# synthesizer-project/synference

Measured on AMD Instinct MI355X. Metric: posterior samples/sec (accepted, prior-box rejection included), higher is better.
Workload: dtype f32

## Files before the change

synference_amd/csrc/sf_api.hip:

```cpp
#include <hip/hip_runtime.h>

#include <chrono>
#include <cmath>
#include <cstdio>
#include <cstdlib>
#include <cstring>
#include <string>
#include <vector>

#include "sf_internal.h"
#include "sf_train.h"
#include "sf_nsf1.h"
#include "sf_nsfar.h"
#include "sf_nsfc.h"
#include "sf_trainc.h"

namespace {
thread_local std::string g_err;

int hip_fail(hipError_t e, const char* what) {
  return sf_fail(SF_ERR_HIP, std::string(what) + ": " + hipGetErrorString(e));
}
}

// ... 209 lines not shown
  add("o_wg0", v.o_wg[0]); add("o_bg0", v.o_bg[0]); add("o_w10", v.o_w1[0]); add("o_b10", v.o_b1[0]);
  add("o_w20", v.o_w2[0]); add("o_b20", v.o_b2[0]); add("o_wg1", v.o_wg[1]); add("o_bg1", v.o_bg[1]);
  add("o_w11", v.o_w1[1]); add("o_b11", v.o_b1[1]); add("o_w21", v.o_w2[1]); add("o_b21", v.o_b2[1]);
  add("o_wout", v.o_wout); add("o_bout", v.o_bout); add("o_lu", v.o_lu);
  add("c_pscale", v.c_pscale); add("c_pshift", v.c_pshift); add("c_tdim", v.c_tdim);
  add("c_xmean", v.c_xmean); add("c_xstd", v.c_xstd); add("c_dslot", v.c_dslot);
  add("nsf_split_sampler", f->L.nsfS.ok); add("trainc_ok", f->L.trc.ok); add("nsfc_ok", f->L.nsc.ok);
  add("inc_ok", v.inc_ok); add("hidden_bf16", v.hidden_bf16); add("tB_stride", v.tB_stride); add("n_parts", v.n_parts); add("part_max", v.part_max);
  add("n_params", f->L.n_params); add("n_packed", f->L.n_packed);
  {
    int R = 0, NV = 0;
    SfDev vv = v;
    vv.packed16 = reinterpret_cast<const float*>(1);
    sf_ctab_shape(vv, R, NV);
    add("ctab_floats_per_galaxy", (long)v.T * NV * R);
  }
  add("o16_w0", v.o16_w0); add("o16_wc", v.o16_wc); add("o16_b0", v.o16_b0); add("o16_wk0", v.o16_wk[0]);
  add("o16_wk1", v.o16_wk[1]); add("o16_bk0", v.o16_bk[0]); add("o16_bk1", v.o16_bk[1]); add("o16_hv", v.o16_hv);
  add("o16_hvb", v.o16_hvb); add("o16_wh", v.o16_wh); add("o16_bh", v.o16_bh); add("o16_wp", v.o16_wp); add("t16_a_tab", v.t16_a_tab);
  add("t16_a", v.t16_a); add("t16B_stride", v.t16B_stride); add("nP16", v.nP16); add("o16B_wk0", v.o16B_wk[0]); add("o16B_wk1", v.o16B_wk[1]);
  add("t16c_stride", v.t16c_stride); add("o16c_bk1", v.o16c_bk1); add("o16c_hvb", v.o16c_hvb); add("o16c_bh", v.o16c_bh);
  add("o16c_wh", v.o16c_wh); add("o16c_wp", v.o16c_wp); add("o16c_blk", v.o16c_blk); add("c16_fix", sf_maf16_compact_fix(v));
  add("sampler_fused", (f->dev_ready && f->ctab_x) ? (sf_maf16_plan(sampler_dev(f, f->ctab_x)).fused ? 1 : 0) : 0);
  add("m16_ok", v.m16_ok); add("m16_span", v.m16_span); add("nT16", v.nT16); add("nC16", v.nC16); add("t16_stride", v.t16_stride);
  s += "\"g16_tile\": [";
  for (int i = 0; i < SF_DMAX; ++i) s += std::to_string(v.g16_tile[i]) + (i + 1 < SF_DMAX ? ", " : "], ");
  s += "\"g16_lo\": [";
  for (int i = 0; i < SF_DMAX; ++i) s += std::to_string(v.g16_lo[i]) + (i + 1 < SF_DMAX ? ", " : "], ");
  s += "\"g_kend\": [";
  for (int i = 0; i < SF_DMAX; ++i) s += std::to_string(v.g_kend[i]) + (i + 1 < SF_DMAX ? ", " : "], ");
  s += "\"g_lo\": [";
  for (int i = 0; i < SF_DMAX; ++i) s += std::to_string(v.g_lo[i]) + (i + 1 < SF_DMAX ? ", " : "], ");
  s += "\"g_tile\": [";
  for (int i = 0; i < SF_DMAX; ++i) s += std::to_string(v.g_tile[i]) + (i + 1 < SF_DMAX ? ", " : "], ");
  s += "\"mt_kend\": [";
  for (int i = 0; i < 4; ++i) s += std::to_string(v.mt_kend[i]) + (i + 1 < 4 ? ", " : "], ");
  s += "\"cst\": [";
  for (size_t i = 0; i < f->L.cst.size(); ++i) {
    char t[40];
    std::snprintf(t, sizeof(t), "%.9g%s", f->L.cst[i], i + 1 < f->L.cst.size() ? ", " : "");
    s += t;
  }
  s += "]}";
  if (s.size() + 1 > buflen) return sf_fail(SF_ERR_INVALID, "buffer too small");
  std::memcpy(buf, s.c_str(), s.size() + 1);
  return SF_OK;
}
// ... 802 lines not shown
```

synference_amd/csrc/sf_layout.cpp:

```cpp
#include "sf_layout.h"

#include <cmath>
#include <cstring>
#include <functional>

namespace {

struct Emitter {
  std::vector<int32_t>& s1;
  std::vector<int32_t>& s2;
  std::vector<int32_t>* gidx = nullptr;
  int64_t cur = 0;

  int64_t pad_to(int64_t align) {
    while (cur % align) push(-1, -1);
    return cur;
  }
  void push(int32_t a, int32_t b, int64_t g = -1) {
    s1.push_back(a);
    s2.push_back(b);
    if (gidx) gidx->push_back((int32_t)(g >= 0 ? g : cur));
    ++cur;
  }
  int64_t linear(int OT, int nG, const std::vector<int>& orow, const std::vector<int>& irow,
// ... 54 lines not shown
  if (d.kind == SF_NSF && (d.K < 2 || d.K > 16)) return fail("K must be in 2..16");
  if (!d.theta_mean || !d.theta_std || !d.x_mean || !d.x_std)
    return fail("z-score buffers must be given");

  const int D = d.D, C = d.C, H = d.H, T = d.T, NB = d.NB, K = d.K;
  SfDev& v = L.dev;
  std::memset(&v, 0, sizeof(v));
  std::memset(&L.trc, 0, sizeof(L.trc));
  std::memset(&L.nsc, 0, sizeof(L.nsc));
  std::memset(&L.nsfS, 0, sizeof(L.nsfS));
  v.kind = d.kind; v.D = D; v.C = C; v.H = H; v.T = T; v.K = K; v.NB = NB;
  v.scale_fn = d.scale_fn;
  v.HT = ceil_div(H, 32);
  v.nGu = ceil_div(D, 8);
  v.nGc = ceil_div(C, 8);
  v.nGh = ceil_div(H, 8);
  v.tail_bound = d.tail_bound; v.min_w = d.min_bin_width; v.min_h = d.min_bin_height;
  v.min_d = d.min_derivative; v.eps = d.maf_eps; v.lu_eps = d.lu_eps;
  v.inv_sqrt_h = (float)(1.0 / std::sqrt((double)H));
  v.deriv_const = (float)std::log(std::exp(1.0 - (double)d.min_derivative) - 1.0);

  std::vector<int> hrow_full(4 * 32, -1);
  std::vector<int> h16row(4 * 16, -1);
  v.inc_ok = 0;
  v.m16_ok = 0;
  if (d.kind == SF_MAF) {
    const int mx = std::max(1, D - 1), mn = std::min(1, D - 1);
    const int G = mx;
    std::vector<std::vector<int>> grp(G);
    for (int j = 0; j < H; ++j) grp[j % mx].push_back(j);
    std::vector<int> rows(4 * 32, -1);
    int tile = 0, used = 0;
    bool ok = true;
    std::vector<int> gt(G), gend(G);
    for (int g = 0; g < G && ok; ++g) {
      const int n = (int)grp[g].size();
      if (n > 32) { ok = false; break; }
      if (used + n > 32) { ++tile; used = 0; }
      if (tile >= 4) { ok = false; break; }
      for (int q = 0; q < n; ++q) rows[tile * 32 + used + q] = grp[g][q];
      used += n;
      gt[g] = tile;
      gend[g] = tile * 32 + used;
    }
    if (ok && D >= 2) {
      const int nGu_e = ceil_div(D, 8), nGc_e = ceil_div(C, 8);
      auto image_floats = [&](int ht, int ngh) {
        return 256L * (ht * (nGu_e + nGc_e) + (long)NB * ht * ngh + ngh) + 64L * D * ht + 64L * (NB + 1) * ht;
// ... 16 lines not shown
      int r = 0;
      for (int g = 0; g < G; ++g) {
        v.g_lo[g + mn] = r / 32;
        for (int j : grp[g]) hrow_full[r++] = j;
        v.g_tile[g + mn] = (r - 1) / 32;
        v.g_kend[g + mn] = ceil_div(r, 8);
      }
      v.inc_ok = (D >= 2 && D <= SF_DMAX && H <= 128) ? 1 : 0;
    }
    {
      h16row.assign(4 * 16, -1);
      int tile16 = 0, used16 = 0;
      bool ok16 = (D >= 2 && NB <= 2);
      for (int g = 0; g < G && ok16; ++g) {
        const int n = (int)grp[g].size();
        if (n > 16) { ok16 = false; break; }
        if (used16 + n > 16) { ++tile16; used16 = 0; }
        if (tile16 >= 4) { ok16 = false; break; }
        for (int q = 0; q < n; ++q) h16row[tile16 * 16 + used16 + q] = grp[g][q];
        used16 += n;
        v.g16_tile[g + mn] = tile16;
      }
      for (int g = 0; g < G; ++g) v.g16_lo[g + mn] = v.g16_tile[g + mn];
      if (!ok16 && D >= 2 && NB <= 2 && H <= 64) {
        h16row.assign(4 * 16, -1);
        int r = 0;
        for (int g = 0; g < G; ++g) {
          v.g16_lo[g + mn] = r / 16;
          for (int j : grp[g]) h16row[r++] = j;
          v.g16_tile[g + mn] = (r - 1) / 16;
        }
        tile16 = (H - 1) / 16;
        ok16 = true;
        v.m16_span = 1;
      }
      v.m16_ok = ok16 ? 1 : 0;
      v.nT16 = ok16 ? tile16 + 1 : 0;
      v.nC16 = ceil_div(C, 16);
    }
  } else {
    for (int j = 0; j < H; ++j) hrow_full[j] = j;
  }
  const int HT = v.HT;
  for (int mt = 0; mt < 4; ++mt) v.mt_kend[mt] = v.nGh;
  if (d.kind == SF_MAF && v.inc_ok) {
    const int mn = std::min(1, D - 1), G = std::max(1, D - 1);
    for (int mt = 0; mt < 4; ++mt) {
      int k = 0;
      for (int g = 0; g < G; ++g)
        if (v.g_lo[g + mn] <= mt && mt <= v.g_tile[g + mn]) k = std::max(k, v.g_kend[g + mn]);
      if (k > 0) v.mt_kend[mt] = k;
    }
  } else if (d.kind == SF_MAF && D >= 2 && H <= 128) {
    const int mx = std::max(1, D - 1);
// ... 276 lines not shown
        if (t == 0) {
          c.ok = 1;
          c.NT = NT;
          std::vector<int> insrc(16, -1);
          int f = 0;
          for (int rho = 0; rho < 16 && f < C; ++rho) {
            const bool slot_row = (rho & 3) < 2 && 2 * (rho >> 2) + (rho & 3) < D;
            if (!slot_row) insrc[rho] = f++;
          }
          while (f < C) {
            for (int rho = 0; rho < 16; ++rho) insrc.push_back(f < C ? f++ : -1);
          }
          c.NI = (int)insrc.size() / 16;
          c.c_insrc = (int)L.cst.size();
          for (int q : insrc) L.cst.push_back((float)q);
          for (int ot = 0; ot < 4; ++ot) { c.kend[ot] = 0; c.kbeg[ot] = NT > 0 ? NT - 1 : 0; }
          c.c_jobs = (int)L.cst.size();
          c.n_jobs = 0;
          for (int ot = 0; ot < NT; ++ot)
            for (int it = 0; it < NT; ++it) {
              bool any = false;
              for (int ro = 0; ro < 16 && !any; ++ro)
                for (int ri = 0; ri < 16 && !any; ++ri) {
                  const int oo = h16row[ot * 16 + ro], ii = h16row[it * 16 + ri];
                  any = oo >= 0 && ii >= 0 && deg_h(oo) >= deg_h(ii);
                }
              if (any) {
                c.kend[ot] = std::max(c.kend[ot], it);
                c.kbeg[it] = std::min(c.kbeg[it], ot);
                L.cst.push_back((float)(ot * 4 + it));
                ++c.n_jobs;
              }
            }
          while (L.cst.size() % 4) L.cst.push_back(0.f);
        }
        const int NI = c.NI;
        auto insrc_at = [&](int it, int rho) { return (int)L.cst[c.c_insrc + it * 16 + rho]; };
        auto pushC = [&](int32_t a, int32_t b) { L.srcC1.push_back(a); L.srcC2.push_back(b); };
        while (L.srcC1.size() % 256) pushC(-1, -1);
        const int64_t tbC = (int64_t)L.srcC1.size();
        if (t == 1) c.t_stride = (int)tbC;
        auto hereC = [&]() { return (int)((int64_t)L.srcC1.size() - tbC); };
        int64_t gcur = 0;
        const int64_t gbase_t = (int64_t)t * c.g_stride;
        auto w_in = [&](int to, int ro, int ti, int ri) -> int64_t {
          const int oo = h16row[to * 16 + ro];
          if (oo < 0) return -1;
          if (ti == 0 && (ri & 3) < 2) {
            const int p = 2 * (ri >> 2) + (ri & 3);
            if (p < D) return deg_h(oo) >= sinv[p] + 1 ? lW0 + (int64_t)oo * D + sinv[p] : -1;
          }
          const int fsrc = insrc_at(ti, ri);
          return fsrc >= 0 ? lWc + (int64_t)oo * C + fsrc : -1;
        };
        auto w_hid = [&](int64_t base) {
          return [&, base](int to, int ro, int ti, int ri) -> int64_t {
            const int oo = h16row[to * 16 + ro], ii = h16row[ti * 16 + ri];
            return (oo >= 0 && ii >= 0 && deg_h(oo) >= deg_h(ii)) ? base + (int64_t)oo * H + ii : -1;
          };
        };
        auto head_row = [&](int ro) -> int {
          const int p = 2 * (ro >> 2) + (ro & 1);
          if (p >= D) return -1;
          return 2 * sinv[p] + ((ro & 3) >= 2 ? 1 : 0);
        };
        auto w_head = [&](int , int ro, int ti, int ri) -> int64_t {
          const int orow_l = head_row(ro), ii = h16row[ti * 16 + ri];
          return (orow_l >= 0 && ii >= 0 && (orow_l / 2 + 1) > deg_h(ii)) ? lWf + (int64_t)orow_l * H + ii : -1;
        };
        using WFn = std::function<int64_t(int, int, int, int)>;
        auto fwd_block = [&](int OT, int IT, const WFn& fn, int64_t g_off) {
          for (int ot = 0; ot < OT; ++ot)
            for (int it = 0; it < IT; ++it)
              for (int l = 0; l < 64; ++l)
                for (int r = 0; r < 4; ++r) {
                  const int ro = l & 15, ri = 4 * (l >> 4) + r;
                  const int64_t idx = fn(ot, ro, it, ri);
                  pushC((int32_t)idx, -1);
                  if (idx >= 0) L.gdstC[(size_t)idx] = (int32_t)(gbase_t + g_off + ((int64_t)ot * IT + it) * 256 + (ro & 3) * 64 + (ro >> 2) * 16 + ri);
                }
        };
        auto tr_block = [&](int ITr, int OTk, const WFn& fn) {
          for (int it = 0; it < ITr; ++it)
            for (int ot = 0; ot < OTk; ++ot)
              for (int l = 0; l < 64; ++l)
                for (int r = 0; r < 4; ++r) pushC((int32_t)fn(ot, 4 * (l >> 4) + r, it, l & 15), -1);
        };
        auto bias_block = [&](int OT, const std::function<int64_t(int, int)>& f1, const std::function<int64_t(int, int)>& f2,
                              int64_t g_off) {
          for (int ot = 0; ot < OT; ++ot)
            for (int ro = 0; ro < 16; ++ro) {
              const int64_t a1 = f1(ot, ro), a2 = f2 ? f2(ot, ro) : -1;
              pushC((int32_t)a1, (int32_t)a2);
              const int32_t g = (int32_t)(gbase_t + g_off + ot * 16 + ro);
              if (a1 >= 0) L.gdstC[(size_t)a1] = g;
              if (a2 >= 0) L.gdstC[(size_t)a2] = g;
            }
        };
        auto hid_bias = [&](int64_t base) {
          return [&, base](int ot, int ro) -> int64_t { const int oo = h16row[ot * 16 + ro]; return oo >= 0 ? base + oo : -1; };
        };
        if (t == 0) L.gdstC.assign((size_t)0, -1);
        if (L.gdstC.size() < (size_t)P) L.gdstC.resize((size_t)P, -1);
        int o; int64_t g;
        o = hereC(); g = gcur; gcur += (int64_t)NT * NI * 256; fwd_block(NT, NI, w_in, g);
        if (t == 0) { c.o_win = o; c.g_win = (int)g; }
        o = hereC(); g = gcur; gcur += NT * 16; bias_block(NT, hid_bias(lb0), hid_bias(lbc), g);
        if (t == 0) { c.o_b0 = o; c.g_b0 = (int)g; }
        o = hereC(); g = gcur; gcur += (int64_t)NT * NT * 256; fwd_block(NT, NT, w_hid(lWk[0]), g);
        if (t == 0) { c.o_w1 = o; c.g_w1 = (int)g; }
        o = hereC(); g = gcur; gcur += NT * 16; bias_block(NT, hid_bias(lbk[0]), nullptr, g);
        if (t == 0) { c.o_b1 = o; c.g_b1 = (int)g; }
        o = hereC(); g = gcur; gcur += (int64_t)NT * NT * 256; fwd_block(NT, NT, w_hid(lWk[1]), g);
        if (t == 0) { c.o_w2 = o; c.g_w2 = (int)g; }
        o = hereC(); g = gcur; gcur += NT * 16; bias_block(NT, hid_bias(lbk[1]), nullptr, g);
        if (t == 0) { c.o_b2 = o; c.g_b2 = (int)g; }
        o = hereC(); g = gcur; gcur += (int64_t)NT * 256; fwd_block(1, NT, w_head, g);
        if (t == 0) { c.o_wf = o; c.g_wf = (int)g; }
        o = hereC(); g = gcur; gcur += 16;
        bias_block(1, [&](int, int ro) -> int64_t { const int r_ = head_row(ro); return r_ >= 0 ? lbf + r_ : -1; }, nullptr, g);
        if (t == 0) { c.o_bf = o; c.g_bf = (int)g; }
        o = hereC(); tr_block(NT, 1, w_head);
        if (t == 0) c.o_wfT = o;
// ... 542 lines not shown
```

synference_amd/csrc/sf_layout.h:

```cpp
#pragma once
#include <cstdint>
#include <string>
#include <vector>

#include "../../include/synference_hip.h"

#define SF_DMAX 16
#define SF_NBMAX 4

struct SfDev {
  const float* packed;
  const float* packedT;
  const float* cst;
  int kind, D, C, H, T, K, NB, scale_fn;
  int HT;
  int PT;
  int KMAX;
  int JP;
  int nGu, nGc, nGh;
  int t_stride;
  int n_parts, part_off[5], part_max;
  int blk_part[SF_NBMAX], head_part;
  int partB_off[5], part_bytes_max;
  int o_w0, o_wc, o_b0;
// ... 10 lines not shown
  int oT_wf, oT_wk[SF_NBMAX], oT_w0;
  int oT_wout, oT_w1[SF_NBMAX], oT_w2[SF_NBMAX], oT_winu;
  int oT_wc;
  int oT_wg[SF_NBMAX];
  int inc_ok;
  int g_tile[SF_DMAX], g_kend[SF_DMAX];
  int g_lo[SF_DMAX];
  int mt_kend[4];
  const unsigned short* packedB;
  int hidden_bf16, nKS, tB_stride;
  int oB_wk[SF_NBMAX], oB_w1[SF_NBMAX], oB_w2[SF_NBMAX];
  const float* packed16;
  int m16_ok, nT16, nC16, t16_stride;
  int t16_a;
  int t16_a_tab;
  int o16_wh, o16_bh;
  int o16_wp;
  const float* packed16c;
  int t16c_stride;
  int o16c_bk1, o16c_hvb, o16c_bh, o16c_wh, o16c_wp, o16c_blk;
  const uint32_t* packed16B;
  int t16B_stride, nP16, o16B_wk[2];
  int m16_span;
  int o16_w0, o16_wc, o16_b0, o16_wk[2], o16_bk[2], o16_hv, o16_hvb;
  int g16_tile[SF_DMAX];
  int g16_lo[SF_DMAX];
  const float* ctab;
  int ctab_R, ctab_NV;
  int c_pscale, c_pshift, c_tdim, c_xmean, c_xstd;
  int c_dslot;
  float logdet0;
  float tail_bound, min_w, min_h, min_d, eps, lu_eps, inv_sqrt_h, deriv_const;
};

#define SF_PACK_TANH_SCALE (-2)
#define SF_PACK_SPLIT_SCALED (1 << 29)
#define SF_PACK_SPLIT_INDEX 0x1fffffff
#define SF_TANH_PRESCALE 2.8853900817779268f

struct SfTrcDev {
  int ok;
  int NT, NI;
  int t_stride, g_stride;
  int o_win, o_b0, o_w1, o_b1, o_w2, o_b2, o_wf, o_bf;
  int o_wfT, o_w2T, o_w1T, o_winT;
  int g_win, g_b0, g_w1, g_b1, g_w2, g_b2, g_wf, g_bf;
// ... 74 lines not shown
```

synference_amd/csrc/sf_maf16.hip:

```cpp
#include "sf_maf16_pass.h"

template <int NB, bool SPAN>
__global__ __launch_bounds__(256, 3) void k_maf_inv16(SfDev m, SfSampleArgsHost a) {
  const int lane = threadIdx.x & 63, wave = threadIdx.x >> 6;
  const int s = lane & 15, g4 = lane >> 4;
  const long item = ((long)blockIdx.x * 4 + wave) * 16 + s;
  const bool valid = item < a.n_items;
  const long it = valid ? item : a.n_items - 1;
  const SfItem16 I = sf_item16(m, a, it, g4);
  f32x4 u = I.u;
  const uint32_t slot = I.slot, att_mine = I.att;
  const long gal = I.gal, ps_idx = I.ps;
  const float* xr = a.x + gal * m.C;
  float logdet = 0.f;

  const float* ctg = (m.ctab && !a.z_in) ? m.ctab + (size_t)gal * m.T * m.ctab_R : nullptr;
  f32x4 ct0;
  if (!ctg) ct0 = sf_ctx_tile16(m, xr, 0, g4);

  const int NT = m.nT16;
  SfPass16 S;
#pragma unroll
  for (int k = 0; k < 3; ++k)
#pragma unroll
// ... 141 lines not shown
           m.o16c_blk == o_blk && m.t16c_stride == size;
  }
  static __device__ __forceinline__ void apply(SfDev& m) {
    m.o16_bk[1] = o_bk1; m.o16_hvb = o_hvb; m.o16_bh = o_bh; m.o16_wh = o_wh; m.o16_wp = o_wp;
  }
};
template <int PREC>
static __host__ __device__ __forceinline__ int sf_lds_floats16(const SfDev& m, bool cp) {
  if constexpr (PREC == 2) return m.t16c_stride + 4 * SF_G16_SCR;
  else return (m.ctab ? m.t16_a_tab : m.t16_a) + SfHid16<PREC>::lds_floats(m, cp);
}
template <int G>
__device__ __forceinline__ void sf_stage16c(const float* src, int wave) {
  const float4* __restrict__ g = reinterpret_cast<const float4*>(src) + (threadIdx.x & 63);
  float4* __restrict__ l = reinterpret_cast<float4*>(sf_lds16);
  for (int gi = __builtin_amdgcn_readfirstlane(wave); gi < G; gi += 4)
    __builtin_amdgcn_global_load_lds((const void*)(g + gi * 64), (void __attribute__((address_space(3)))*)(l + gi * 64), 16, 0, 0);
  __builtin_amdgcn_s_waitcnt(0x0f70);
}

#ifndef SF_SAMP16_WG_FUSED
#define SF_SAMP16_WG_FUSED 4
#endif
template <int NB, bool SPAN, bool HM, int DD = 0, int PREC = 0>
__global__ __launch_bounds__(256, (SPAN ? 3 : (PREC == 2 ? SF_SAMP16_WG_FUSED : 4))) void k_maf_samp16(SfSamp16Args args_in) {
  static_assert(DD == 0 || (HM && !SPAN && DD >= 2 && DD <= 5), "unrolled passes: head tile, aligned placement, D <= 5");
  static_assert(PREC != 2 || DD >= 3, "fused first layer: unrolled kernels only (m_fix and the compact image's offsets)");
  using HID = SfHid16<PREC>;
  constexpr int TPW = SF_SAMP16_TPW;
  constexpr int IPW = 64 * TPW;
  const int wave = threadIdx.x >> 6;
  using FC = SfFixC16<NB, (PREC == 2 ? DD : 2)>;
  unsigned int* ctrl = reinterpret_cast<unsigned int*>(sf_lds16 + sf_lds_floats16<PREC>(args_in.m, !SPAN));
  unsigned int pf;
  sf_q_begin<IPW>(args_in.a, ctrl, pf);
  float* ecb = reinterpret_cast<float*>(ctrl + SF_Q_WORDS(IPW));
  sf_ecb16_build<true>(ecb, args_in.m, args_in.a);
#ifdef SF_Q_STATS
  const unsigned long long qs_k0 = __builtin_amdgcn_s_memtime();
  unsigned long long qs_iters = 0, qs_last_work = 0;
  unsigned long long qs_ph[10] = {0, 0, 0, 0, 0, 0, 0, 0, 0, 0};
  if (threadIdx.x == 0) atomicMin(&args_in.a.q->stats[10], __builtin_amdgcn_s_memrealtime());
#endif
  for (;;) {
    const SfSamp16Args* ap;
    {
      auto kp = __builtin_amdgcn_kernarg_segment_ptr();
      asm volatile("" : "+s"(kp));
// ... 67 lines not shown
      { const unsigned long long n = __builtin_amdgcn_s_memrealtime(); qs_ph[qs_o + (t == m.T - 1 ? 1 : 3)] += n - qs_t_mark; qs_t_mark = n; }
#endif
      __syncthreads();
      if constexpr (PREC == 2) sf_stage16c<FC::groups>(m.packed16c + (size_t)t * FC::size, wave);
      else sf_stage16<PREC, !SPAN>(m, t, S.tab ? m.t16_a_tab : m.t16_a, wave);
      __syncthreads();
#ifdef SF_Q_STATS
      { const unsigned long long n = __builtin_amdgcn_s_memrealtime(); qs_ph[qs_o + 2] += n - qs_t_mark; qs_t_mark = n; }
#endif
      const float* tp = sf_lds16;
      const void* tpB = sf_lds16 + (PREC == 2 ? FC::o_blk : (S.tab ? m.t16_a_tab : m.t16_a));
#pragma unroll 1
      for (int j = 0; j < TPW; ++j) {
        const bool tile_has_work = (unsigned)((j * 4 + wave) * 16) < n_items;
        if (tile_has_work) {
          if (j > 0) {
            S.c0p = S.tab ? m.ctab + ((size_t)gal_cur * m.T + t) * m.ctab_R + (PREC == 2 ? m.nT16 * 16 : 0) : nullptr;
            if constexpr (PREC == 2) sf_pre16g_load<DD - 1>(S, g4);
            else if (HM && S.tab) sf_c0_prefetch(S, tiles.tile(2), g4);
          }
          if (HM) S.hdone = sf_ld4(tp + m.o16_bh + g4 * 4);
          if constexpr (PREC == 2) {
            float* scr = sf_lds16 + FC::size + wave * SF_G16_SCR + s * SF_G16_ROW;
            sf_transform16g<NB, DD>(m, tp, static_cast<const float*>(tpB), S, dsl, u_cur, scr, lane, g4);
          } else {
            S.xr = a.x + gal_cur * m.C;
            if constexpr (DD > 0) {
              sf_transform16s<HID, NB, DD>(m, tp, tpB, S, NT, dsl, u_cur, lane, g4);
            } else {
              HID::template clear<false, HM>(S);
#pragma unroll
              for (int r = 0; r < 4; ++r) S.ut[r] = 0.f;
              {
                const int sl = __builtin_amdgcn_readlane(dsl, 0);
                sf_pass16_deg1(m, tp, S.ut, sl, sf_slot16_own(u_cur, sl), g4);
              }
              for (int p = 2; p <= m.D; ++p) {
                const int sl = __builtin_amdgcn_readlane(dsl, p - 1);
                sf_pass16_tiles<HID, NB, SPAN, HM>(m, tp, tpB, S, NT, tiles, p, m.D, sl, sf_slot16_own(u_cur, sl), lane, g4);
              }
              u_cur = S.ut;
            }
          }
        }
        if (TPW > 1) {
          const f32x4 tu = u_t[0];
          const unsigned int tg = g_t[0];
// ... 85 lines not shown
      const unsigned int n_ev = (unsigned)__popcll(__ballot(valid && g4 == 0));
      const unsigned int n_r0 = (unsigned)__popcll(__ballot(leader && first < 0 && att_base == 0u));
      if ((threadIdx.x & 63) == 0) {
        if (n_res) atomicAdd(&ctrl[4], n_res);
        if (n_ev) atomicAdd(&ctrl[5], n_ev);
        if (n_r0) atomicAdd(&ctrl[6], n_r0);
      }
      if (TPW > 1) {
        const f32x4 tu = u_t[0];
#pragma unroll
        for (int q = 0; q + 1 < TPW; ++q) u_t[q] = u_t[q + 1];
        u_t[TPW - 1] = tu;
      }
    }
#ifdef SF_Q_STATS
    qs_last_work = __builtin_amdgcn_s_memrealtime();
    qs_ph[qs_o + 4] += qs_last_work - qs_t_mark;
    if (a.qtrace && threadIdx.x == 0 && qs_iters <= (2048u * 256u) / gridDim.x)
      a.qtrace[((size_t)blockIdx.x * ((2048u * 256u) / gridDim.x) + qs_iters - 1) * 4 + 3] = (uint32_t)qs_last_work;
#endif
  }
}

template <int NB, int DD, int PREC = 0>
__global__ __launch_bounds__(256, 4) void k_maf_find16s(SfDev m, SfSampleArgsHost a) {
  using HID = SfHid16<PREC>;
  using FC = SfFixC16<NB, DD>;
  SfFix16<NB, DD>::apply(m);
  const int lane = threadIdx.x & 63, wave = threadIdx.x >> 6;
  const int s = lane & 15, g4 = lane >> 4;
  float* ecb = sf_lds16 + sf_lds_floats16<PREC>(m, true);
  sf_ecb16_build<false>(ecb, m, a);
  if constexpr (PREC == 2) FC::apply(m);
  const int NT = m.nT16;
  f32x4 u_cur, u_oth;
  long gal_cur = 0, gal_oth = 0;
#pragma unroll
  for (int j = 1; j >= 0; --j) {
    const long item = ((long)blockIdx.x * 8 + j * 4 + wave) * 16 + s;
    const long it = item < a.n_items ? item : a.n_items - 1;
    const SfItem16 I = sf_item16(m, a, it, g4);
    if (j == 1) { u_oth = I.u; gal_oth = I.gal; }
    else { u_cur = I.u; gal_cur = I.gal; }
  }
  typename HID::State S;
  S.tab = true;
  if constexpr (PREC != 2) S.xr = nullptr;
  for (int t = m.T - 1; t >= 0; --t) {
    const int dsl = (int)m.cst[m.c_dslot + t * SF_DMAX + s];
    S.c0p = m.ctab + ((size_t)gal_cur * m.T + t) * m.ctab_R + (PREC == 2 ? m.nT16 * 16 : 0);
    if constexpr (PREC == 2) sf_pre16g_load<DD - 1>(S, g4);
    else sf_c0_prefetch(S, 0, g4);
    __syncthreads();
    if constexpr (PREC == 2) sf_stage16c<FC::groups>(m.packed16c + (size_t)t * FC::size, wave);
    else sf_stage16<PREC, true>(m, t, m.t16_a_tab, wave);
    __syncthreads();
    const float* tp = sf_lds16;
    const void* tpB = sf_lds16 + (PREC == 2 ? FC::o_blk : m.t16_a_tab);
#pragma unroll 1
    for (int j = 0; j < 2; ++j) {
      if (((long)blockIdx.x * 8 + j * 4 + wave) * 16 < a.n_items) {
        if (j > 0) {
          S.c0p = m.ctab + ((size_t)gal_cur * m.T + t) * m.ctab_R + (PREC == 2 ? m.nT16 * 16 : 0);
          if constexpr (PREC == 2) sf_pre16g_load<DD - 1>(S, g4);
          else sf_c0_prefetch(S, 0, g4);
        }
        S.hdone = sf_ld4(tp + m.o16_bh + g4 * 4);
        if constexpr (PREC == 2) {
          float* scr = sf_lds16 + FC::size + wave * SF_G16_SCR + s * SF_G16_ROW;
          sf_transform16g<NB, DD>(m, tp, static_cast<const float*>(tpB), S, dsl, u_cur, scr, lane, g4);
        } else {
          sf_transform16s<HID, NB, DD>(m, tp, tpB, S, NT, dsl, u_cur, lane, g4);
        }
      }
      { const f32x4 tu = u_cur; u_cur = u_oth; u_oth = tu; }
      { const long tg = gal_cur; gal_cur = gal_oth; gal_oth = tg; }
    }
  }
#pragma unroll 1
  for (int j = 0; j < 2; ++j) {
    const long item = ((long)blockIdx.x * 8 + j * 4 + wave) * 16 + s;
    const bool valid = item < a.n_items;
    const long it = valid ? item : a.n_items - 1;
    const long ps = it >> a.log2_attempts;
    const uint32_t att = a.att_list ? a.att_list[ps] : a.attempt + (uint32_t)(it & ((1L << a.log2_attempts) - 1));
    float th[4];
    int tdc[4];
    bool ok = sf_theta_box16(ecb, u_cur, g4, th, tdc);
    if (a.att_list && att == 0xffffffffu) ok = false;
    const uint32_t acc16 = sf_accept16(ok, valid);
    const bool accepted = (acc16 >> s) & 1u;
    if (a.z_in) {
      if (valid) {
// ... 64 lines not shown
  return m.D == 3 ? SfFixC16<2, 3>::matches(m) : (m.D == 4 ? SfFixC16<2, 4>::matches(m) : SfFixC16<2, 5>::matches(m));
}
static int sf_maf16_seq_d(const SfDev& m) {
  if (!m.ctab || m.m16_span || m.D < 3 || m.D > 5 || m.nT16 != m.D - 1) return 0;
  for (int p = 2; p <= m.D; ++p)
    if (m.g16_tile[p - 1] != p - 2) return 0;
  bool fits = false;
  if (m.NB == 1) fits = m.D == 3 ? SfFix16<1, 3>::matches(m) : (m.D == 4 ? SfFix16<1, 4>::matches(m) : SfFix16<1, 5>::matches(m));
  else if (m.NB == 2) fits = m.D == 3 ? SfFix16<2, 3>::matches(m) : (m.D == 4 ? SfFix16<2, 4>::matches(m) : SfFix16<2, 5>::matches(m));
  return fits ? m.D : 0;
}
SfMaf16Plan sf_maf16_plan(const SfDev& m) {
  SfMaf16Plan pl;
  pl.fp32 = sf_sampler_fp32_for(SF_MAF) != 0;
  pl.ok16 = m.kind == SF_MAF && m.m16_ok && !m.hidden_bf16 && m.packed16 != nullptr;
  pl.sampler16 = pl.ok16 && (m.packed16B != nullptr || pl.fp32);
  pl.span = m.m16_span != 0;
  pl.head_mfma = !m.m16_span && m.o16_wh >= 0;
  pl.dd = pl.head_mfma ? sf_maf16_seq_d(m) : 0;
  pl.fused = pl.dd > 0 && pl.fp32 && m.o16_wp >= 0 && m.ctab_R == 2 * m.nT16 * 16 && m.packed16c != nullptr && sf_maf16_compact_fix(m) == 1;
  return pl;
}

template <int NB, int DD, int PREC>
static hipError_t sf_launch_find16s(const SfDev& m, const SfSampleArgsHost& a, hipStream_t st) {
  static SfAttrCache attr;
  const size_t sh = (size_t)sf_lds_floats16<PREC>(m, true) * sizeof(float) + 80 * sizeof(float);
  if (hipError_t e = sf_lds_optin16(k_maf_find16s<NB, DD, PREC>, attr); e != hipSuccess) return e;
  hipLaunchKernelGGL((k_maf_find16s<NB, DD, PREC>), dim3((unsigned)((a.n_items + 127) / 128)), dim3(256), sh, st, m, a);
  return hipGetLastError();
}

template <int NB, bool SPAN, bool HM, int PREC = 0>
__global__ __launch_bounds__(256, 3) void k_maf_inv16b(SfDev m, const float* __restrict__ z, const float* __restrict__ x,
                                                       long n, float* __restrict__ out) {
  using HID = SfHid16<PREC>;
  const int lane = threadIdx.x & 63, wave = threadIdx.x >> 6;
  const int s = lane & 15, g4 = lane >> 4;
  const long item = ((long)blockIdx.x * 4 + wave) * 16 + s;
  const bool valid = item < n;
  const long it = valid ? item : n - 1;
  f32x4 u;
#pragma unroll
  for (int r = 0; r < 4; ++r) u[r] = (4 * g4 + r < m.D) ? z[it * m.D + 4 * g4 + r] : 0.f;
  const int NT = m.nT16;
  SfTiles16 tiles;
  tiles.pack(m);
  typename HID::State S;
  HID::template clear<false, false>(S);
  for (int t = m.T - 1; t >= 0; --t) {
    __syncthreads();
    sf_stage16<PREC, !SPAN>(m, t, m.t16_a, wave);
// ... 127 lines not shown
  hipLaunchKernelGGL(k_maf_compact16, dim3((unsigned)m.T), dim3(256), 0, st, m, tab, out);
  return hipGetLastError();
}
hipError_t sf_launch_maf_ctab16(const SfDev& m, const float* x, long M, float* tab, hipStream_t st) {
  hipLaunchKernelGGL(k_maf_ctab16, dim3((unsigned)((M + 63) / 64), (unsigned)m.T), dim3(256), 0, st, m, x, M, tab);
  return hipGetLastError();
}

bool sf_maf16_enabled(const SfDev& m, const SfSampleArgsHost& a) {
  return sf_maf16_plan(m).ok16 && (a.attempts_per_slot <= 16 || a.best != nullptr);
}

static int sf_resident_blocks16(const void* fn, size_t sh, int cap) {
  int dev = 0, cus = 256, per = cap;
  if (hipGetDevice(&dev) == hipSuccess) {
    hipDeviceProp_t pr;
    if (hipGetDeviceProperties(&pr, dev) == hipSuccess && pr.multiProcessorCount > 0) cus = pr.multiProcessorCount;
  }
  int occ = 0;
  if (hipOccupancyMaxActiveBlocksPerMultiprocessor(&occ, fn, 256, sh) == hipSuccess && occ > 0) per = occ < cap ? occ : cap;
  return cus * per;
}

template <int NB, bool SPAN, bool HM, int DD, int PREC>
static hipError_t sf_launch16q_p(const SfDev& m, const SfSampleArgsHost& a, hipStream_t st) {
  static SfAttrCache attr;
  static SfResidentCache rcache;
  const size_t sh = (size_t)sf_lds_floats16<PREC>(m, !SPAN) * sizeof(float) + (SF_Q_WORDS(64 * SF_SAMP16_TPW) + 96) * sizeof(unsigned int);
  if (sh > 160 * 1024) return hipErrorInvalidValue;
  if (hipError_t e = sf_lds_optin16(k_maf_samp16<NB, SPAN, HM, DD, PREC>, attr); e != hipSuccess) return e;
  int resident = 0, cur_dev = 0;
  (void)hipGetDevice(&cur_dev);
  if (!rcache.get(cur_dev, sh, resident)) {
    resident = sf_resident_blocks16((const void*)k_maf_samp16<NB, SPAN, HM, DD, PREC>, sh, SPAN ? 3 : (PREC == 2 ? SF_SAMP16_WG_FUSED : 4));
    rcache.put(cur_dev, sh, resident);
  }
  long grid = (a.n_items + 64 * SF_SAMP16_TPW - 1) / (64 * SF_SAMP16_TPW);
  if (grid > resident) grid = resident;
  SfSamp16Args args;
  args.m = m;
  args.a = a;
  hipLaunchKernelGGL((k_maf_samp16<NB, SPAN, HM, DD, PREC>), dim3((unsigned)grid), dim3(256), sh, st, args);
  return hipGetLastError();
}
template <int NB, bool SPAN, bool HM, int DD>
static hipError_t sf_launch16q(const SfDev& m, const SfSampleArgsHost& a, const SfMaf16Plan& pl, hipStream_t st) {
  if constexpr (DD > 0) {
    if (pl.fused) return sf_launch16q_p<NB, SPAN, HM, DD, 2>(m, a, st);
  }
  if (pl.fp32) return sf_launch16q_p<NB, SPAN, HM, DD, 1>(m, a, st);
  if (!m.packed16B) return hipErrorInvalidValue;
  return sf_launch16q_p<NB, SPAN, HM, DD, 0>(m, a, st);
}
template <int NB, bool SPAN>
static hipError_t sf_launch16(const SfDev& m, const SfSampleArgsHost& a, hipStream_t st) {
  static SfAttrCache attr;
  const size_t sh = (size_t)m.t16_stride * sizeof(float);
  if (hipError_t e = sf_lds_optin16(k_maf_inv16<NB, SPAN>, attr); e != hipSuccess) return e;
  const long per_block = 4L * 16;
  hipLaunchKernelGGL((k_maf_inv16<NB, SPAN>), dim3((unsigned)((a.n_items + per_block - 1) / per_block)), dim3(256), sh, st, m, a);
  return hipGetLastError();
}
static hipError_t sf_launch_find16(const SfDev& m, const SfSampleArgsHost& a, const SfMaf16Plan& pl, hipStream_t st) {
  return sf_visit_unrolled16(m.NB, pl.dd, [&](auto nb, auto dd) {
    return pl.fused ? sf_launch_find16s<nb(), dd(), 2>(m, a, st)
                    : (pl.fp32 ? sf_launch_find16s<nb(), dd(), 1>(m, a, st) : sf_launch_find16s<nb(), dd(), 0>(m, a, st));
  });
}
hipError_t sf_launch_maf_find16_zin(const SfDev& m, const SfSampleArgsHost& a, hipStream_t st) {
  const SfMaf16Plan pl = sf_maf16_plan(m);
  return pl.fused ? sf_launch_find16(m, a, pl, st) : hipErrorInvalidValue;
}
hipError_t sf_launch_maf_inv16(const SfDev& m, const SfSampleArgsHost& a, hipStream_t st) {
  const SfMaf16Plan pl = sf_maf16_plan(m);
  if (a.q) {
    if (pl.dd > 0)
      return sf_visit_unrolled16(m.NB, pl.dd, [&](auto nb, auto dd) { return sf_launch16q<nb(), false, true, dd()>(m, a, pl, st); });
    return sf_visit_shape16(m.NB, pl.span, pl.head_mfma,
                            [&](auto nb, auto sp, auto hm) { return sf_launch16q<nb(), sp(), hm(), 0>(m, a, pl, st); });
  }
  if ((a.best || a.att_list || a.count) && !a.z_in && pl.dd > 0 && (pl.fp32 || m.packed16B)) return sf_launch_find16(m, a, pl, st);
  return sf_visit_shape16(m.NB, pl.span, false, [&](auto nb, auto sp, auto) { return sf_launch16<nb(), sp()>(m, a, st); });
}
```

synference_amd/csrc/sf_maf16_pass.h:

```cpp
#pragma once
#include <hip/hip_runtime.h>

#include <type_traits>

#include "sf_device.h"
#include "sf_internal.h"
#include "sf_rng.h"

typedef float f32x4 __attribute__((ext_vector_type(4)));
typedef float f32x2 __attribute__((ext_vector_type(2)));
#define SF_MFMA16(a, b, c) __builtin_amdgcn_mfma_f32_16x16x4f32((a), (b), (c), 0, 0, 0)

__device__ __forceinline__ float sf_sum4groups(float v) {
  v += __shfl_xor(v, 16, 64);
  v += __shfl_xor(v, 32, 64);
  return v;
}
__device__ __forceinline__ f32x4 sf_mma16(float4 w, const f32x4& in, f32x4 acc) {
  acc = SF_MFMA16(w.x, in[0], acc);
  acc = SF_MFMA16(w.y, in[1], acc);
  acc = SF_MFMA16(w.z, in[2], acc);
  acc = SF_MFMA16(w.w, in[3], acc);
  return acc;
}
// ... 536 lines not shown
template <int NT>
__device__ __forceinline__ void sf_pre16g_load(SfPass16G& S, int g4) {
#pragma unroll
  for (int ot = 0; ot < NT; ++ot) S.pre[ot] = *reinterpret_cast<const f32x4*>(S.c0p + ot * 16 + 4 * g4);
}
__device__ __forceinline__ f32x4 sf_rank1(const f32x4& acc, const float4& w, float v) {
  const f32x2 vv = {v, v};
  const f32x2 lo = __builtin_elementwise_fma(f32x2{w.x, w.y}, vv, f32x2{acc[0], acc[1]});
  const f32x2 hi = __builtin_elementwise_fma(f32x2{w.z, w.w}, vv, f32x2{acc[2], acc[3]});
  return f32x4{lo[0], lo[1], hi[0], hi[1]};
}
template <int NT, int K>
struct SfWpCols {
  float4 w[NT - K + 1];
  __device__ __forceinline__ void load(const float* tp, int o_wp, int g4) {
#pragma unroll
    for (int q = 0; q <= NT - K; ++q) w[q] = *reinterpret_cast<const float4*>(tp + o_wp + sf_wp16_entry(NT, K, K - 1 + q) * 16 + 4 * g4);
  }
  __device__ __forceinline__ void apply(SfPass16G& S, float wv) const {
#pragma unroll
    for (int q = 0; q <= NT - K; ++q) S.pre[K - 1 + q] = sf_rank1(S.pre[K - 1 + q], w[q], wv);
  }
};
template <int OT, int NB, int NT>
__device__ __forceinline__ float sf_pass16g(const SfDev& m, const float* tp, const float* tpF, SfPass16G& S, int sl, float u_in,
                                            int lane, int g4) {
  const float4 wh = sf_w16(tp + m.o16_wh, NT, 0, OT, lane);
  float4 fw[OT + 1];
  f32x4 b1;
  if (NB == 2) {
    b1 = sf_ld4(tp + m.o16_bk[1] + (OT * 4 + g4) * 4);
#pragma unroll
    for (int it = 0; it <= OT; ++it) fw[it] = sf_w16f<true>(tpF, NT, OT, it, lane);
  }
  SfWpCols<NT, (OT + 2 <= NT ? OT + 2 : NT)> wu;
  if constexpr (OT + 2 <= NT) wu.load(tp, m.o16_wp, g4);
  __builtin_amdgcn_sched_barrier(0);
  if (NB == 2) {
#pragma unroll
    for (int it = 0; it < OT; ++it) b1 = sf_mma16(fw[it], S.act[it], b1);
  }
  f32x4 last = sf_tanh4(S.pre[OT]);
  if (NB == 2) {
    S.act[OT] = last;
    b1 = sf_mma16(fw[OT], last, b1);
    last = sf_tanh4(b1);
  }
  S.hdone = sf_mma16(wh, last, S.hdone);
  const bool odd = (sl & 1) != 0;
  const int src = (lane & 15) + 16 * (sl >> 1);
  const float av = __shfl(odd ? S.hdone[2] : S.hdone[0], src, 64);
  const float mv = __shfl(odd ? S.hdone[3] : S.hdone[1], src, 64);
  const float wv = sf_div(u_in - mv, sf_scale16(m, av));
  if constexpr (OT + 2 <= NT) wu.apply(S, wv);
  return wv;
}
template <int NB, int DD>
__device__ __forceinline__ void sf_transform16g(const SfDev& m, const float* tp, const float* tpF, SfPass16G& S, int dsl, f32x4& u,
                                                float* scr, int lane, int g4) {
  constexpr int NT = DD - 1;
  *reinterpret_cast<f32x4*>(scr + 4 * g4) = u;
  int sl[DD];
  float ud[DD];
#pragma unroll
  for (int q = 0; q < DD; ++q) {
    sl[q] = __builtin_amdgcn_readlane(dsl, q);
    ud[q] = scr[sl[q]];
  }
  {
    SfWpCols<NT, 1> wu;
    wu.load(tp, m.o16_wp, g4);
    const float av = tp[m.o16_hvb + 2 * sl[0]], mv = tp[m.o16_hvb + 2 * sl[0] + 1];
    const float wv = sf_div(ud[0] - mv, sf_scale16(m, av));
    wu.apply(S, wv);
    scr[sl[0]] = wv;
  }
  auto pass = [&](auto otc) {
    constexpr int OT = decltype(otc)::value;
    scr[sl[OT + 1]] = sf_pass16g<OT, NB, NT>(m, tp, tpF, S, sl[OT + 1], ud[OT + 1], lane, g4);
  };
  pass(std::integral_constant<int, 0>{});
  if constexpr (DD >= 3) pass(std::integral_constant<int, 1>{});
  if constexpr (DD >= 4) pass(std::integral_constant<int, 2>{});
  if constexpr (DD >= 5) pass(std::integral_constant<int, 3>{});
  u = *reinterpret_cast<const f32x4*>(scr + 4 * g4);
}
template <> struct SfHid16<2> {
  using State = SfPass16G;
};

__device__ __forceinline__ void sf_copy_group16(const float4* g, float4* l) {
  __builtin_amdgcn_global_load_lds((const void*)g, (void __attribute__((address_space(3)))*)l, 16, 0, 0);
  __builtin_amdgcn_global_load_lds((const void*)g, (void __attribute__((address_space(3)))*)l, 16, 1024, 0);
  __builtin_amdgcn_global_load_lds((const void*)g, (void __attribute__((address_space(3)))*)l, 16, 2048, 0);
  __builtin_amdgcn_global_load_lds((const void*)g, (void __attribute__((address_space(3)))*)l, 16, 3072, 0);
}

template <int PREC, bool CP>
__device__ __forceinline__ void sf_stage16(const SfDev& m, int t, int a_floats, int wave) {
  const int lane_ = threadIdx.x & 63;
  const int ga = a_floats >> 10;
  const float4* __restrict__ sa = reinterpret_cast<const float4*>(m.packed16 + (size_t)t * m.t16_stride);
// ... 149 lines not shown
```

Baseline: 1.108 billion.

## Pack hidden rows into three k-slots per tile to skip fourth MFMA k-step

When each hidden group of the MAF fits one 16-row tile with at most 12 rows, rows are re-placed so the fourth k-slot of every 4-row block is empty. The fused sampler and find kernels get a K3 template parameter that drops the last MFMA k-step and one tanh lane for those tiles. This cuts matrix and transcendental work in the sequential autoregressive passes. The cost is extra kernel instantiations, and correctness relies on the packed-weight builder still using the original row map while the kernel uses the new placement.

Result: faster. 1.165 billion (median of 6 runs) (+5.2%).

```diff
diff --git a/synference_amd/csrc/sf_api.hip b/synference_amd/csrc/sf_api.hip
--- a/synference_amd/csrc/sf_api.hip
+++ b/synference_amd/csrc/sf_api.hip
@@ -255,7 +255,7 @@
   add("t16c_stride", v.t16c_stride); add("o16c_bk1", v.o16c_bk1); add("o16c_hvb", v.o16c_hvb); add("o16c_bh", v.o16c_bh);
   add("o16c_wh", v.o16c_wh); add("o16c_wp", v.o16c_wp); add("o16c_blk", v.o16c_blk); add("c16_fix", sf_maf16_compact_fix(v));
   add("sampler_fused", (f->dev_ready && f->ctab_x) ? (sf_maf16_plan(sampler_dev(f, f->ctab_x)).fused ? 1 : 0) : 0);
-  add("m16_ok", v.m16_ok); add("m16_span", v.m16_span); add("nT16", v.nT16); add("nC16", v.nC16); add("t16_stride", v.t16_stride);
+  add("m16_ok", v.m16_ok); add("m16_span", v.m16_span); add("m16_k3", v.m16_k3); add("nT16", v.nT16); add("nC16", v.nC16); add("t16_stride", v.t16_stride);
   s += "\"g16_tile\": [";
   for (int i = 0; i < SF_DMAX; ++i) s += std::to_string(v.g16_tile[i]) + (i + 1 < SF_DMAX ? ", " : "], ");
   s += "\"g16_lo\": [";
diff --git a/synference_amd/csrc/sf_layout.cpp b/synference_amd/csrc/sf_layout.cpp
--- a/synference_amd/csrc/sf_layout.cpp
+++ b/synference_amd/csrc/sf_layout.cpp
@@ -100,8 +100,10 @@
 
   std::vector<int> hrow_full(4 * 32, -1);
   std::vector<int> h16row(4 * 16, -1);
+  std::vector<int> h16row_trc;
   v.inc_ok = 0;
   v.m16_ok = 0;
+  v.m16_k3 = 0;
   if (d.kind == SF_MAF) {
     const int mx = std::max(1, D - 1), mn = std::min(1, D - 1);
     const int G = mx;
@@ -164,6 +166,21 @@
         v.g16_tile[g + mn] = tile16;
       }
       for (int g = 0; g < G; ++g) v.g16_lo[g + mn] = v.g16_tile[g + mn];
+      h16row_trc = h16row;
+      if (ok16 && D >= 3 && D <= 5 && tile16 + 1 == D - 1) {
+        bool one_per_tile = true;
+        for (int g = 0; g < G; ++g) one_per_tile = one_per_tile && v.g16_tile[g + mn] == g;
+        if (one_per_tile) {
+          std::vector<int> ks(G);
+          for (int g = 0; g < G; ++g) {
+            const int n = (int)grp[g].size();
+            ks[g] = std::max(3, ceil_div(n, 4));
+            for (int r = 0; r < 16; ++r) h16row[g * 16 + r] = -1;
+            for (int q = 0; q < n; ++q) h16row[g * 16 + 4 * (q / ks[g]) + q % ks[g]] = grp[g][q];
+          }
+          while (v.m16_k3 < G && ks[G - 1 - v.m16_k3] == 3) ++v.m16_k3;
+        }
+      }
       if (!ok16 && D >= 2 && NB <= 2 && H <= 64) {
         h16row.assign(4 * 16, -1);
         int r = 0;
@@ -172,6 +189,7 @@
           for (int j : grp[g]) h16row[r++] = j;
           v.g16_tile[g + mn] = (r - 1) / 16;
         }
+        h16row_trc = h16row;
         tile16 = (H - 1) / 16;
         ok16 = true;
         v.m16_span = 1;
@@ -494,7 +512,7 @@
               bool any = false;
               for (int ro = 0; ro < 16 && !any; ++ro)
                 for (int ri = 0; ri < 16 && !any; ++ri) {
-                  const int oo = h16row[ot * 16 + ro], ii = h16row[it * 16 + ri];
+                  const int oo = h16row_trc[ot * 16 + ro], ii = h16row_trc[it * 16 + ri];
                   any = oo >= 0 && ii >= 0 && deg_h(oo) >= deg_h(ii);
                 }
               if (any) {
@@ -516,7 +534,7 @@
         int64_t gcur = 0;
         const int64_t gbase_t = (int64_t)t * c.g_stride;
         auto w_in = [&](int to, int ro, int ti, int ri) -> int64_t {
-          const int oo = h16row[to * 16 + ro];
+          const int oo = h16row_trc[to * 16 + ro];
           if (oo < 0) return -1;
           if (ti == 0 && (ri & 3) < 2) {
             const int p = 2 * (ri >> 2) + (ri & 3);
@@ -527,7 +545,7 @@
         };
         auto w_hid = [&](int64_t base) {
           return [&, base](int to, int ro, int ti, int ri) -> int64_t {
-            const int oo = h16row[to * 16 + ro], ii = h16row[ti * 16 + ri];
+            const int oo = h16row_trc[to * 16 + ro], ii = h16row_trc[ti * 16 + ri];
             return (oo >= 0 && ii >= 0 && deg_h(oo) >= deg_h(ii)) ? base + (int64_t)oo * H + ii : -1;
           };
         };
@@ -537,7 +555,7 @@
           return 2 * sinv[p] + ((ro & 3) >= 2 ? 1 : 0);
         };
         auto w_head = [&](int , int ro, int ti, int ri) -> int64_t {
-          const int orow_l = head_row(ro), ii = h16row[ti * 16 + ri];
+          const int orow_l = head_row(ro), ii = h16row_trc[ti * 16 + ri];
           return (orow_l >= 0 && ii >= 0 && (orow_l / 2 + 1) > deg_h(ii)) ? lWf + (int64_t)orow_l * H + ii : -1;
         };
         using WFn = std::function<int64_t(int, int, int, int)>;
@@ -570,7 +588,7 @@
             }
         };
         auto hid_bias = [&](int64_t base) {
-          return [&, base](int ot, int ro) -> int64_t { const int oo = h16row[ot * 16 + ro]; return oo >= 0 ? base + oo : -1; };
+          return [&, base](int ot, int ro) -> int64_t { const int oo = h16row_trc[ot * 16 + ro]; return oo >= 0 ? base + oo : -1; };
         };
         if (t == 0) L.gdstC.assign((size_t)0, -1);
         if (L.gdstC.size() < (size_t)P) L.gdstC.resize((size_t)P, -1);
diff --git a/synference_amd/csrc/sf_layout.h b/synference_amd/csrc/sf_layout.h
--- a/synference_amd/csrc/sf_layout.h
+++ b/synference_amd/csrc/sf_layout.h
@@ -56,6 +56,7 @@
   const uint32_t* packed16B;
   int t16B_stride, nP16, o16B_wk[2];
   int m16_span;
+  int m16_k3;
   int o16_w0, o16_wc, o16_b0, o16_wk[2], o16_bk[2], o16_hv, o16_hvb;
   int g16_tile[SF_DMAX];
   int g16_lo[SF_DMAX];
diff --git a/synference_amd/csrc/sf_maf16.hip b/synference_amd/csrc/sf_maf16.hip
--- a/synference_amd/csrc/sf_maf16.hip
+++ b/synference_amd/csrc/sf_maf16.hip
@@ -187,8 +187,9 @@
 #ifndef SF_SAMP16_WG_FUSED
 #define SF_SAMP16_WG_FUSED 4
 #endif
-template <int NB, bool SPAN, bool HM, int DD = 0, int PREC = 0>
+template <int NB, bool SPAN, bool HM, int DD = 0, int PREC = 0, int K3 = 0>
 __global__ __launch_bounds__(256, (SPAN ? 3 : (PREC == 2 ? SF_SAMP16_WG_FUSED : 4))) void k_maf_samp16(SfSamp16Args args_in) {
+  static_assert(K3 == 0 || (PREC == 2 && K3 <= DD - 1), "skipped k-steps: the fused passes only, at most every hidden tile");
   static_assert(DD == 0 || (HM && !SPAN && DD >= 2 && DD <= 5), "unrolled passes: head tile, aligned placement, D <= 5");
   static_assert(PREC != 2 || DD >= 3, "fused first layer: unrolled kernels only (m_fix and the compact image's offsets)");
   using HID = SfHid16<PREC>;
@@ -302,7 +303,7 @@
           if (HM) S.hdone = sf_ld4(tp + m.o16_bh + g4 * 4);
           if constexpr (PREC == 2) {
             float* scr = sf_lds16 + FC::size + wave * SF_G16_SCR + s * SF_G16_ROW;
-            sf_transform16g<NB, DD>(m, tp, static_cast<const float*>(tpB), S, dsl, u_cur, scr, lane, g4);
+            sf_transform16g<NB, DD, K3>(m, tp, static_cast<const float*>(tpB), S, dsl, u_cur, scr, lane, g4);
           } else {
             S.xr = a.x + gal_cur * m.C;
             if constexpr (DD > 0) {
@@ -434,8 +435,9 @@
   }
 }
 
-template <int NB, int DD, int PREC = 0>
+template <int NB, int DD, int PREC = 0, int K3 = 0>
 __global__ __launch_bounds__(256, 4) void k_maf_find16s(SfDev m, SfSampleArgsHost a) {
+  static_assert(K3 == 0 || (PREC == 2 && K3 <= DD - 1), "skipped k-steps: the fused passes only");
   using HID = SfHid16<PREC>;
   using FC = SfFixC16<NB, DD>;
   SfFix16<NB, DD>::apply(m);
@@ -480,7 +482,7 @@
         S.hdone = sf_ld4(tp + m.o16_bh + g4 * 4);
         if constexpr (PREC == 2) {
           float* scr = sf_lds16 + FC::size + wave * SF_G16_SCR + s * SF_G16_ROW;
-          sf_transform16g<NB, DD>(m, tp, static_cast<const float*>(tpB), S, dsl, u_cur, scr, lane, g4);
+          sf_transform16g<NB, DD, K3>(m, tp, static_cast<const float*>(tpB), S, dsl, u_cur, scr, lane, g4);
         } else {
           sf_transform16s<HID, NB, DD>(m, tp, tpB, S, NT, dsl, u_cur, lane, g4);
         }
@@ -591,12 +593,24 @@
   return pl;
 }
 
-template <int NB, int DD, int PREC>
+template <int DD, typename F>
+static hipError_t sf_visit_k3(int k3, F&& f) {
+  switch (k3) {
+    case 0: return f(std::integral_constant<int, 0>{});
+    case 1: return f(std::integral_constant<int, 1>{});
+    case 2: return f(std::integral_constant<int, 2>{});
+    case 3: if constexpr (DD >= 4) return f(std::integral_constant<int, 3>{}); else return hipErrorInvalidValue;
+    case 4: if constexpr (DD >= 5) return f(std::integral_constant<int, 4>{}); else return hipErrorInvalidValue;
+    default: return hipErrorInvalidValue;
+  }
+}
+
+template <int NB, int DD, int PREC, int K3 = 0>
 static hipError_t sf_launch_find16s(const SfDev& m, const SfSampleArgsHost& a, hipStream_t st) {
   static SfAttrCache attr;
   const size_t sh = (size_t)sf_lds_floats16<PREC>(m, true) * sizeof(float) + 80 * sizeof(float);
-  if (hipError_t e = sf_lds_optin16(k_maf_find16s<NB, DD, PREC>, attr); e != hipSuccess) return e;
-  hipLaunchKernelGGL((k_maf_find16s<NB, DD, PREC>), dim3((unsigned)((a.n_items + 127) / 128)), dim3(256), sh, st, m, a);
+  if (hipError_t e = sf_lds_optin16(k_maf_find16s<NB, DD, PREC, K3>, attr); e != hipSuccess) return e;
+  hipLaunchKernelGGL((k_maf_find16s<NB, DD, PREC, K3>), dim3((unsigned)((a.n_items + 127) / 128)), dim3(256), sh, st, m, a);
   return hipGetLastError();
 }
 
@@ -770,17 +784,17 @@
   return cus * per;
 }
 
-template <int NB, bool SPAN, bool HM, int DD, int PREC>
+template <int NB, bool SPAN, bool HM, int DD, int PREC, int K3 = 0>
 static hipError_t sf_launch16q_p(const SfDev& m, const SfSampleArgsHost& a, hipStream_t st) {
   static SfAttrCache attr;
   static SfResidentCache rcache;
   const size_t sh = (size_t)sf_lds_floats16<PREC>(m, !SPAN) * sizeof(float) + (SF_Q_WORDS(64 * SF_SAMP16_TPW) + 96) * sizeof(unsigned int);
   if (sh > 160 * 1024) return hipErrorInvalidValue;
-  if (hipError_t e = sf_lds_optin16(k_maf_samp16<NB, SPAN, HM, DD, PREC>, attr); e != hipSuccess) return e;
+  if (hipError_t e = sf_lds_optin16(k_maf_samp16<NB, SPAN, HM, DD, PREC, K3>, attr); e != hipSuccess) return e;
   int resident = 0, cur_dev = 0;
   (void)hipGetDevice(&cur_dev);
   if (!rcache.get(cur_dev, sh, resident)) {
-    resident = sf_resident_blocks16((const void*)k_maf_samp16<NB, SPAN, HM, DD, PREC>, sh, SPAN ? 3 : (PREC == 2 ? SF_SAMP16_WG_FUSED : 4));
+    resident = sf_resident_blocks16((const void*)k_maf_samp16<NB, SPAN, HM, DD, PREC, K3>, sh, SPAN ? 3 : (PREC == 2 ? SF_SAMP16_WG_FUSED : 4));
     rcache.put(cur_dev, sh, resident);
   }
   long grid = (a.n_items + 64 * SF_SAMP16_TPW - 1) / (64 * SF_SAMP16_TPW);
@@ -788,13 +802,13 @@
   SfSamp16Args args;
   args.m = m;
   args.a = a;
-  hipLaunchKernelGGL((k_maf_samp16<NB, SPAN, HM, DD, PREC>), dim3((unsigned)grid), dim3(256), sh, st, args);
+  hipLaunchKernelGGL((k_maf_samp16<NB, SPAN, HM, DD, PREC, K3>), dim3((unsigned)grid), dim3(256), sh, st, args);
   return hipGetLastError();
 }
 template <int NB, bool SPAN, bool HM, int DD>
 static hipError_t sf_launch16q(const SfDev& m, const SfSampleArgsHost& a, const SfMaf16Plan& pl, hipStream_t st) {
   if constexpr (DD > 0) {
-    if (pl.fused) return sf_launch16q_p<NB, SPAN, HM, DD, 2>(m, a, st);
+    if (pl.fused) return sf_visit_k3<DD>(m.m16_k3, [&](auto k3) { return sf_launch16q_p<NB, SPAN, HM, DD, 2, k3()>(m, a, st); });
   }
   if (pl.fp32) return sf_launch16q_p<NB, SPAN, HM, DD, 1>(m, a, st);
   if (!m.packed16B) return hipErrorInvalidValue;
@@ -811,8 +825,9 @@
 }
 static hipError_t sf_launch_find16(const SfDev& m, const SfSampleArgsHost& a, const SfMaf16Plan& pl, hipStream_t st) {
   return sf_visit_unrolled16(m.NB, pl.dd, [&](auto nb, auto dd) {
-    return pl.fused ? sf_launch_find16s<nb(), dd(), 2>(m, a, st)
-                    : (pl.fp32 ? sf_launch_find16s<nb(), dd(), 1>(m, a, st) : sf_launch_find16s<nb(), dd(), 0>(m, a, st));
+    constexpr int NB_ = decltype(nb)::value, DD_ = decltype(dd)::value;
+    if (pl.fused) return sf_visit_k3<DD_>(m.m16_k3, [&](auto k3) { return sf_launch_find16s<NB_, DD_, 2, k3()>(m, a, st); });
+    return (pl.fp32 ? sf_launch_find16s<nb(), dd(), 1>(m, a, st) : sf_launch_find16s<nb(), dd(), 0>(m, a, st));
   });
 }
 hipError_t sf_launch_maf_find16_zin(const SfDev& m, const SfSampleArgsHost& a, hipStream_t st) {
diff --git a/synference_amd/csrc/sf_maf16_pass.h b/synference_amd/csrc/sf_maf16_pass.h
--- a/synference_amd/csrc/sf_maf16_pass.h
+++ b/synference_amd/csrc/sf_maf16_pass.h
@@ -582,9 +582,31 @@
     for (int q = 0; q <= NT - K; ++q) S.pre[K - 1 + q] = sf_rank1(S.pre[K - 1 + q], w[q], wv);
   }
 };
-template <int OT, int NB, int NT>
+template <bool SKIP>
+__device__ __forceinline__ f32x4 sf_mma16k(float4 w, const f32x4& in, f32x4 acc) {
+  acc = SF_MFMA16(w.x, in[0], acc);
+  acc = SF_MFMA16(w.y, in[1], acc);
+  acc = SF_MFMA16(w.z, in[2], acc);
+  if constexpr (!SKIP) acc = SF_MFMA16(w.w, in[3], acc);
+  return acc;
+}
+template <bool SKIP>
+__device__ __forceinline__ f32x4 sf_tanh4k(const f32x4& b) {
+  if constexpr (!SKIP) {
+    return sf_tanh4(b);
+  } else {
+    const f32x2 one = {1.0f, 1.0f}, m2 = {-2.0f, -2.0f};
+    const f32x2 e01 = f32x2{__builtin_amdgcn_exp2f(b[0]), __builtin_amdgcn_exp2f(b[1])} + one;
+    const float e2 = __builtin_amdgcn_exp2f(b[2]) + 1.0f;
+    const f32x2 r01 = {__builtin_amdgcn_rcpf(e01[0]), __builtin_amdgcn_rcpf(e01[1])};
+    const f32x2 o01 = __builtin_elementwise_fma(r01, m2, one);
+    return f32x4{o01[0], o01[1], __builtin_fmaf(__builtin_amdgcn_rcpf(e2), -2.0f, 1.0f), 0.f};
+  }
+}
+template <int OT, int NB, int NT, int K3 = 0>
 __device__ __forceinline__ float sf_pass16g(const SfDev& m, const float* tp, const float* tpF, SfPass16G& S, int sl, float u_in,
                                             int lane, int g4) {
+  constexpr bool SK = OT >= NT - K3;
   const float4 wh = sf_w16(tp + m.o16_wh, NT, 0, OT, lane);
   float4 fw[OT + 1];
   f32x4 b1;
@@ -598,15 +620,15 @@
   __builtin_amdgcn_sched_barrier(0);
   if (NB == 2) {
 #pragma unroll
-    for (int it = 0; it < OT; ++it) b1 = sf_mma16(fw[it], S.act[it], b1);
-  }
-  f32x4 last = sf_tanh4(S.pre[OT]);
+    for (int it = 0; it < OT; ++it) b1 = it >= NT - K3 ? sf_mma16k<true>(fw[it], S.act[it], b1) : sf_mma16k<false>(fw[it], S.act[it], b1);
+  }
+  f32x4 last = sf_tanh4k<SK>(S.pre[OT]);
   if (NB == 2) {
     S.act[OT] = last;
-    b1 = sf_mma16(fw[OT], last, b1);
-    last = sf_tanh4(b1);
-  }
-  S.hdone = sf_mma16(wh, last, S.hdone);
+    b1 = sf_mma16k<SK>(fw[OT], last, b1);
+    last = sf_tanh4k<SK>(b1);
+  }
+  S.hdone = sf_mma16k<SK>(wh, last, S.hdone);
   const bool odd = (sl & 1) != 0;
   const int src = (lane & 15) + 16 * (sl >> 1);
   const float av = __shfl(odd ? S.hdone[2] : S.hdone[0], src, 64);
@@ -615,7 +637,7 @@
   if constexpr (OT + 2 <= NT) wu.apply(S, wv);
   return wv;
 }
-template <int NB, int DD>
+template <int NB, int DD, int K3 = 0>
 __device__ __forceinline__ void sf_transform16g(const SfDev& m, const float* tp, const float* tpF, SfPass16G& S, int dsl, f32x4& u,
                                                 float* scr, int lane, int g4) {
   constexpr int NT = DD - 1;
@@ -637,7 +659,7 @@
   }
   auto pass = [&](auto otc) {
     constexpr int OT = decltype(otc)::value;
-    scr[sl[OT + 1]] = sf_pass16g<OT, NB, NT>(m, tp, tpF, S, sl[OT + 1], ud[OT + 1], lane, g4);
+    scr[sl[OT + 1]] = sf_pass16g<OT, NB, NT, K3>(m, tp, tpF, S, sl[OT + 1], ud[OT + 1], lane, g4);
   };
   pass(std::integral_constant<int, 0>{});
   if constexpr (DD >= 3) pass(std::integral_constant<int, 1>{});
```
